# EllarBooher/Syzygy

Measured on AMD Instinct MI355X. Metric: Mpixels/s deferred-lit+atmosphere, higher is better.
Workload: dtype f32

## Files before the change

syzygy_amd/csrc/api_skyview.cpp:

```cpp

#include <new>

#include "api_common.hpp"
#include "lut_state.hpp"
#include "szg/multiscatter_sky.h"

using namespace szg;

struct szg_skyview
{
    int device = 0;
    szg_skyview_desc desc{};
    DeviceBuffer<float> d_transmittance, d_skyview, d_multiscatter, d_aerialLuminance, d_aerialTransmittance;
    float aerialMaxDistance = 0.0f;
    uint32_t multiscatter = SZG_MULTISCATTER_OFF;
    mutable LutState luts;
    DeviceBuffer<unsigned> d_slutStatusAll;
    bool lutReuse = false;
    DeviceBuffer<unsigned> d_lutKey;
    DeviceBuffer<void> d_framePrep;
    DeviceBuffer<void> d_framePrepDraw;
};

static hipError_t ensure_tlut_status(szg_skyview* p, hipStream_t s)
// ... 33 lines not shown

int szg_skyview_create(szg_skyview_t** out, const szg_skyview_desc* desc, int device)
{
    if (out == nullptr)
    {
        return fail(SZG_ERR_INVALID_ARGUMENT, "szg_skyview_create: out is NULL");
    }
    *out = nullptr;
    szg_skyview_desc d{512u, 128u, 2048u, 1024u, 0u, 0u};
    if (desc != nullptr)
    {
        d = *desc;
    }
    if (d.transmittance_width < 2u || d.transmittance_height < 2u || d.skyview_width < 2u || d.skyview_height < 2u ||
        d.transmittance_width > 16384u || d.transmittance_height > 16384u || d.skyview_width > 16384u ||
        d.skyview_height > 16384u)
    {
        return fail(SZG_ERR_INVALID_ARGUMENT, "szg_skyview_create: LUT extents out of range");
    }
    if (d.flags != 0u)
    {
        return fail(SZG_ERR_INVALID_ARGUMENT, "szg_skyview_create: unknown flags 0x%x", d.flags);
    }
    SZG_TRY_RC(select_device(device));
    szg_skyview* p = new (std::nothrow) szg_skyview();
    if (p == nullptr)
    {
        return fail(SZG_ERR_OUT_OF_MEMORY, "szg_skyview_create: host allocation failed");
    }
    p->device = device;
    p->desc = d;
#define SZG_TRY(expr) SZG_HIP_OR(expr, szg_skyview_destroy(p), "szg_skyview_create: hipMalloc")
    size_t const aerialTexels = (size_t)SZG_AERIAL_W * SZG_AERIAL_H * SZG_AERIAL_D;
    SZG_TRY(p->d_transmittance.alloc(tlut_block_bytes(d.transmittance_width, d.transmittance_height) / sizeof(float)));
    SZG_TRY(p->d_skyview.alloc(slut_block_bytes(d.skyview_width, d.skyview_height) / sizeof(float)));
    SZG_TRY(p->d_multiscatter.alloc((size_t)SZG_MULTISCATTER_DIM * SZG_MULTISCATTER_DIM * 4u));
    SZG_TRY(p->d_aerialLuminance.alloc(aerialTexels * 4u));
    SZG_TRY(p->d_aerialTransmittance.alloc(aerialTexels * 4u));
    SZG_TRY(p->d_lutKey.alloc(LUT_KEY_DWORDS, true));
    SZG_TRY(p->d_framePrep.alloc(frame_prep_bytes()));
    SZG_TRY(p->d_slutStatusAll.alloc(SLUT_STATUS_RANKS));
    SZG_TRY(p->d_framePrepDraw.alloc(frame_prep_bytes()));
#undef SZG_TRY
    *out = p;
    return SZG_OK;
}

int szg_skyview_set_lut_reuse(szg_skyview_t* p, int enable)
{
    if (p == nullptr)
    {
        return fail(SZG_ERR_INVALID_ARGUMENT, "szg_skyview_set_lut_reuse: NULL argument");
    }
    p->lutReuse = enable != 0;
    p->luts.reuse_switched();
    return SZG_OK;
}

int szg_skyview_set_multiscatter(szg_skyview_t* p, uint32_t mode)
{
    if (p == nullptr || mode > SZG_MULTISCATTER_ONLY)
    {
        return fail(SZG_ERR_INVALID_ARGUMENT, "szg_skyview_set_multiscatter: NULL pipeline or unknown mode %u", mode);
    }
    if (mode != p->multiscatter)
    {
        p->multiscatter = mode;
// ... 48 lines not shown
    *out = make_image(p->d_transmittance, p->desc.transmittance_width, p->desc.transmittance_height, SZG_FORMAT_RGBA32_SFLOAT);
    p->luts.transmittance_exposed();
    return SZG_OK;
}

int szg_skyview_skyview_lut(const szg_skyview_t* p, szg_image* out)
{
    if (p == nullptr || out == nullptr)
    {
        return fail(SZG_ERR_INVALID_ARGUMENT, "szg_skyview_skyview_lut: NULL argument");
    }
    *out = make_image(p->d_skyview, p->desc.skyview_width, p->desc.skyview_height, SZG_FORMAT_RGBA32_SFLOAT);
    p->luts.skyview_exposed();
    return SZG_OK;
}

int szg_skyview_record_transmittance(szg_skyview_t* p, void* stream, uint32_t atmosphere_index,
                                     const szg_atmosphere_packed* d_atmospheres)
{
    if (p == nullptr || d_atmospheres == nullptr)
    {
        return fail(SZG_ERR_INVALID_ARGUMENT, "szg_skyview_record_transmittance: NULL argument");
    }
    DeviceGuard const guard(p->device);
    hipStream_t const s = static_cast<hipStream_t>(stream);
    const unsigned* dirty = nullptr;
    if (p->lutReuse)
    {
        SZG_HIP(szg::launch_lut_key(s, d_atmospheres, atmosphere_index, nullptr, 0u, p->d_lutKey, 0u, p->luts.forceTransmittance,
                                    p->d_transmittance, p->desc.transmittance_width, p->desc.transmittance_height));
        dirty = p->d_lutKey + 69;
    }
    SZG_HIP(szg::launch_transmittance(s, d_atmospheres, atmosphere_index, p->d_transmittance, p->desc.transmittance_width,
                                      p->desc.transmittance_height, dirty));
    p->luts.transmittance_recorded();
    return SZG_OK;
}

int szg_skyview_record_skyview_lut_rows(szg_skyview_t* p, void* stream, uint32_t atmosphere_index,
                                        const szg_atmosphere_packed* d_atmospheres, uint32_t view_camera_index,
                                        const szg_camera_packed* d_cameras, uint32_t row_begin, uint32_t row_end)
{
    if (p == nullptr || d_atmospheres == nullptr || d_cameras == nullptr)
    {
        return fail(SZG_ERR_INVALID_ARGUMENT, "szg_skyview_record_skyview_lut_rows: NULL argument");
    }
    if (row_begin > row_end || row_end > p->desc.skyview_height)
    {
        return fail(SZG_ERR_INVALID_ARGUMENT, "szg_skyview_record_skyview_lut_rows: rows [%u, %u) outside the %u-row LUT", row_begin,
                    row_end, p->desc.skyview_height);
    }
    if (!multiscatter_ready(p, "szg_skyview_record_skyview_lut_rows"))
    {
        return SZG_ERR_INVALID_ARGUMENT;
    }
    DeviceGuard const guard(p->device);
    hipStream_t const s = static_cast<hipStream_t>(stream);
    bool const whole = LutState::whole(row_begin, row_end, p->desc.skyview_height);
    SZG_HIP(ensure_tlut_status(p, s));
    const unsigned* dirty = nullptr;
    if (p->lutReuse && whole)
    {
        SZG_HIP(szg::launch_lut_key(s, d_atmospheres, atmosphere_index, d_cameras, view_camera_index, p->d_lutKey, 1u, p->luts.forceSkyview,
                                    p->d_skyview, p->desc.skyview_width, p->desc.skyview_height));
        dirty = p->d_lutKey + 70;
    }
    SZG_HIP(szg::launch_frame_prep(s, d_atmospheres, atmosphere_index, p->desc.transmittance_width, p->desc.transmittance_height,
                                   p->d_framePrep));
    if (p->multiscatter == SZG_MULTISCATTER_OFF)
    {
        SZG_HIP(szg::launch_skyview(s, d_atmospheres, atmosphere_index, d_cameras, view_camera_index, p->d_transmittance,
                                    p->desc.transmittance_width, p->desc.transmittance_height, p->d_skyview, p->desc.skyview_width,
                                    p->desc.skyview_height, row_begin, row_end, dirty, p->d_framePrep));
    }
    else
    {
        SZG_HIP(szg::launch_skyview_ms(s, p->multiscatter, d_atmospheres, atmosphere_index, d_cameras, view_camera_index,
                                       p->d_transmittance, p->desc.transmittance_width, p->desc.transmittance_height,
                                       p->d_multiscatter, p->d_skyview, p->desc.skyview_width, p->desc.skyview_height, row_begin,
                                       row_end, dirty, p->d_framePrep));
    }
    p->luts.skyview_rows_recorded(row_begin, row_end, p->desc.skyview_height);
    return SZG_OK;
}

int szg_skyview_lut_row_slice(const szg_skyview_t* p, uint32_t rank, uint32_t nranks, uint32_t* row_begin, uint32_t* row_end)
{
    if (p == nullptr || row_begin == nullptr || row_end == nullptr || nranks == 0u || rank >= nranks)
    {
        return fail(SZG_ERR_INVALID_ARGUMENT, "szg_skyview_lut_row_slice: NULL argument or rank outside [0, nranks)");
    }
    if (p->desc.skyview_height % nranks != 0u)
    {
        return fail(SZG_ERR_INVALID_ARGUMENT, "szg_skyview_lut_row_slice: %u LUT rows do not divide over %u ranks", p->desc.skyview_height,
                    nranks);
    }
    uint32_t const n = p->desc.skyview_height / nranks;
    *row_begin = rank * n;
    *row_end = (rank + 1u) * n;
    return SZG_OK;
}

int szg_skyview_allgather_lut_rows(szg_skyview_t* p, szg_rowtile_comm_t* comm, void* stream)
{
    if (p == nullptr || comm == nullptr)
    {
        return fail(SZG_ERR_INVALID_ARGUMENT, "szg_skyview_allgather_lut_rows: NULL argument");
    }
    int const nranks = szg_rowtile_comm_size(comm);
    if (nranks < 1 || p->desc.skyview_height % (uint32_t)nranks != 0u)
    {
        return fail(SZG_ERR_INVALID_ARGUMENT, "szg_skyview_allgather_lut_rows: %u LUT rows do not divide over %d ranks",
                    p->desc.skyview_height, nranks);
// ... 212 lines not shown
```

syzygy_amd/csrc/kernels_lut.hip:

```cpp

#include "szg/fpmath.h"
#include "szg_atmosphere.hpp"
#include "szg_launch.hpp"
#include "szg_lean.hpp"
#include "szg_lut_rays.hpp"
#include "szg_march.hpp"
#include "szg_vec.hpp"

namespace szg
{
template <int CTRL> SZG_DEV float dpp(float v)
{
    return __builtin_bit_cast(float, __builtin_amdgcn_update_dpp(0, __builtin_bit_cast(int, v), CTRL, 0xF, 0xF, false));
}

constexpr int T_LANES = 8;
constexpr int T_STEPS = 500;

template <bool LEAN> SZG_DEV V3 transmittanceProduct(const Atm& a, V3 origin, V3 direction, float distance, float ndt, int sub)
{
    V3 T = splat(1.0f);
    float const rcp500 = rcpN(500.0f);
#pragma unroll 1
    for (int k = 0; k < (T_STEPS + T_LANES - 1) / T_LANES; k++)
    {
        int const i = k * T_LANES + sub;
        float const t = divRX<LEAN>(distance * ((float)i + 0.5f), 500.0f, rcp500);
        V3 const position = origin + t * direction;
        float const altitude = sqrtPX<LEAN>(dotT(position, position)) - a.planetRadius;
        Extinction const e = sampleExtinction<LEAN>(a, altitude);
        bool const valid = i < T_STEPS;
        float const fx = valid ? expX<LEAN>(ndt * e.extinction.x) : 1.0f;
        float const fy = valid ? expX<LEAN>(ndt * e.extinction.y) : 1.0f;
        float const fz = valid ? expX<LEAN>(ndt * e.extinction.z) : 1.0f;
        T.x = dpp<0x107>(T.x) * fx;
        T.y = dpp<0x107>(T.y) * fy;
        T.z = dpp<0x107>(T.z) * fz;
#pragma unroll
        for (int j = 1; j < T_LANES; j++)
        {
            T.x = dpp<0x111>(T.x) * fx;
            T.y = dpp<0x111>(T.y) * fy;
            T.z = dpp<0x111>(T.z) * fz;
        }
    }
    return T;
}

__global__ __launch_bounds__(256) void k_transmittance(const szg_atmosphere_packed* __restrict__ atmospheres,
                                                      unsigned atmosphereIndex, float4* __restrict__ lut, int W, int H,
                                                      const unsigned* __restrict__ dirty)
{
    if (dirty != nullptr && dirty[0] == 0u)
    {
        return;
    }
    int const sub = (int)(threadIdx.x & (unsigned)(T_LANES - 1));
    int const idRaw = (int)((blockIdx.x * 256u + threadIdx.x) / (unsigned)T_LANES);
    bool const inRangeTexel = idRaw < W * H;
    int const id = inRangeTexel ? idRaw : (W * H - 1);
    int const tx = id % W;
    int const ty = id / W;
    Atm const a = load_atm(atmospheres + atmosphereIndex);

    float const u = ((float)tx + 0.5f) / (float)W;
    float const v = ((float)ty + 0.5f) / (float)H;

    float const x_mu = (u - 0.5f / (float)W) / (1.0f - 1.0f / (float)W);
    float const x_radius = (v - 0.5f / (float)H) / (1.0f - 1.0f / (float)H);
    float const rho = a.H * x_radius;
    float const radius = sqrtf(rho * rho + a.Rp2);
    float const d_min = a.atmosphereRadius - radius;
    float const d_max = rho + a.H;
    float const d = (d_max - d_min) * x_mu + d_min;
    float mu = 1.0f;
    if (d != 0.0f)
    {
        mu = clampf((a.H * a.H - rho * rho - d * d) / (2.0f * radius * d), -1.0f, 1.0f);
    }

    V3 const origin = mk3(0.0f, radius, 0.0f);
    V3 const direction = mk3(sqrtf(1.0f - mu * mu), mu, 0.0f);

    float t0 = 0.0f, t1 = 0.0f;
    bool const hit = raySphere(origin, direction, a.atmosphereRadius, t0, t1);
    float const distance = hit ? t1 : 0.0f;
    float const dt = distance / 500.0f;
    float const ndt = -fabsf(dt);
    float const rmin2 = mu < 0.0f ? radius * radius * (1.0f - mu * mu) : radius * radius;
    bool const lean = waveAll(a.lean && rmin2 >= a.leanFloor2 && inRange(radius, 0x1p-30f, 0x1p30f) && inRange(distance, 0.0f, 0x1p30f));
    V3 const T = lean ? transmittanceProduct<true>(a, origin, direction, distance, ndt, sub)
                      : transmittanceProduct<false>(a, origin, direction, distance, ndt, sub);
    if (inRangeTexel && sub == T_LANES - 1)
    {
        float4 const texel = hit ? make_float4(T.x, T.y, T.z, 1.0f) : make_float4(1.0f, 1.0f, 1.0f, 1.0f);
        lut[id] = texel;
        if (!tlutTexelModerate(texel.x, texel.y, texel.z))
        {
            atomicOr(reinterpret_cast<unsigned*>(lut + (size_t)W * (size_t)H), 1u);
        }
    }
}

__global__ __launch_bounds__(256) void k_lut_range(float4* __restrict__ lut, unsigned n)
{
    unsigned const id = blockIdx.x * 256u + threadIdx.x;
    bool ok = true;
    if (id < n)
    {
        float4 const t = lut[id];
        ok = tlutTexelModerate(t.x, t.y, t.z);
    }
    if (!waveAll(ok) && (threadIdx.x & 63u) == 0u)
    {
        atomicOr(reinterpret_cast<unsigned*>(lut + n), 1u);
    }
}

__global__ __launch_bounds__(64) void k_frame_prep(const szg_atmosphere_packed* __restrict__ atmospheres, unsigned atmosphereIndex,
                                                   int tW, int tH, FramePrep* __restrict__ out,
                                                   const szg_directional_light_packed* __restrict__ sun,
                                                   const szg_camera_packed* __restrict__ cameras, unsigned cameraIndex, unsigned drawW,
                                                   unsigned drawH)
{
    if (threadIdx.x != 0u)
    {
        return;
    }
    FramePrep f{};
    f.a = load_atm(atmospheres + atmosphereIndex);
    f.fwidth = (float)tW;
    f.fheight = (float)tH;
    f.u_bias = 0.5f / (float)tW;
    f.u_scale = 1.0f - 1.0f / (float)tW;
    f.v_bias = 0.5f / (float)tH;
    f.v_scale = 1.0f - 1.0f / (float)tH;
    {
        auto vOf = [&](float x_radius) {
            float const t = SZG_CON(SZG_C_LUTMAP, x_radius, f.v_scale, f.v_bias);
            return SZG_CON(SZG_C_TEXCOORD, t, f.fheight, -0.5f);
        };
        float const rMax = sqrtf(f.a.innerCeil2) * (1.0f + 0x1p-16f);
        float const rhoMax = safeSqrt(rMax * rMax - f.a.Rp2);
        float const vLo = vOf(0.0f), vHi = vOf(rhoMax / f.a.H);
        bool const ok = f.a.lean && vLo >= 0.0f && floorf(vHi) + 1.0f <= f.fheight - 1.0f && vHi == vHi && tW >= 2 && tH >= 2 &&
                        (float)tW * (float)tH <= 0x1p24f;
        f.rowsInterior = ok ? 1u : 0u;
    }
#pragma unroll
    for (int k = 0; k < 16; k++)
    {
        f.sunShadow[k] = 0.0f;
    }
    if (sun != nullptr)
    {
        M4 toTex;
        float const t[16] = {0.5f, 0.0f, 0.0f, 0.0f, 0.0f, 0.5f, 0.0f, 0.0f, 0.0f, 0.0f, 1.0f, 0.0f, 0.5f, 0.5f, 0.0f, 1.0f};
#pragma unroll
        for (int k = 0; k < 16; k++)
        {
// ... 15 lines not shown
        position.y *= -1.0f;
        position.y += f.a.planetRadius;
        c.position = position;
        c.r2 = dot(position, position);
        c.sinHorizon = f.a.planetRadius / length(position);
        c.horizonZenith = PI - szg_asinf(c.sinHorizon);
        c.cosHorizonZenith = -safeSqrt(1.0f - c.sinHorizon * c.sinHorizon);
        c.piMinusHorizon = PI - c.horizonZenith;
        V3 const directionToSun = -f.a.incidentDirectionSun;
        c.projectedLight = normalize(V2{-f.a.incidentDirectionSun.x, -f.a.incidentDirectionSun.z});
        c.sunLength = length(directionToSun);
        c.lightDirection = normalize(directionToSun);
        TLut L{};
        L.width = tW;
        L.height = tH;
        L.fwidth = f.fwidth;
        L.fheight = f.fheight;
        L.u_bias = f.u_bias;
        L.u_scale = f.u_scale;
        L.v_bias = f.v_bias;
        L.v_scale = f.v_scale;
        c.lenFrom = lengthA(position);
        RadiusPart const p = radiusPart<false>(L, f.a, c.lenFrom);
        c.from_r2 = p.r2;
        c.from_d_min = p.d_min;
        c.from_denom = p.denom;
        c.from_rcpDenom = rcpN(p.denom);
        c.from_b = p.b;
        c.from_omb = p.omb;
        c.from_row0 = p.row0;
        c.from_row1 = p.row1;
        c.rcpDrawW = rcpN((float)drawW);
        c.rcpDrawH = rcpN((float)drawH);
    }
    *out = f;
}

__global__ __launch_bounds__(256, 4) void k_skyview(const szg_atmosphere_packed* __restrict__ atmospheres, unsigned atmosphereIndex,
                                                 const szg_camera_packed* __restrict__ cameras, unsigned cameraIndex,
                                                 const float4* __restrict__ tlut, int tW, int tH, float4* __restrict__ lut,
                                                 int W, int H, int rowBegin, int rowEnd, const unsigned* __restrict__ dirty,
                                                 const FramePrep* __restrict__ prep)
{
    if (dirty != nullptr && dirty[0] == 0u)
    {
        return;
    }
    unsigned const tid = threadIdx.x;
    unsigned const wave = tid >> 6, lane = tid & 63u;
    int const x = (int)(blockIdx.x * 32u + wave * 8u + (lane & 7u));
    int const y = rowBegin + (int)(blockIdx.y * 8u + (lane >> 3));
    if (x >= W || y >= rowEnd)
    {
        return;
    }
    Atm const a = load_atm(*prep);
    TLut const L = make_tlut(tlut, tW, tH, *prep);
    const szg_camera_packed* cam = cameras + cameraIndex;
    V3 origin, direction;
    skyviewTexelRay(a, cam, x, y, W, H, origin, direction);

    float const distance = raycastAtmosphere(a, origin, direction);
    V3 const luminance = scatteringIntegral(L, a, origin, direction, distance);
    lut[y * W + x] = make_float4(luminance.x, luminance.y, luminance.z, 1.0f);
    if (!slutTexelFinite(luminance.x, luminance.y, luminance.z))
    {
        atomicOr(reinterpret_cast<unsigned*>(lut + (size_t)W * (size_t)H), 1u);
    }
}

__global__ __launch_bounds__(256) void k_slut_check(float4* __restrict__ lut, unsigned n)
{
    unsigned const id = blockIdx.x * 256u + threadIdx.x;
    bool ok = true;
    if (id < n)
    {
        float4 const t = lut[id];
        ok = slutTexelFinite(t.x, t.y, t.z);
    }
    if (!waveAll(ok) && (threadIdx.x & 63u) == 0u)
    {
        atomicOr(reinterpret_cast<unsigned*>(lut + n), 1u);
    }
}

__global__ void k_slut_status_stage(unsigned* __restrict__ all, unsigned rank, const unsigned* __restrict__ status, unsigned known)
{
    if (threadIdx.x == 0u)
    {
        all[rank] = known != 0u ? status[0] : 1u;
    }
}
__global__ void k_slut_status_reduce(const unsigned* __restrict__ all, unsigned nranks, unsigned* __restrict__ status)
// ... 105 lines not shown
    {
        V3 const pg = pos + tMax * dir;
        V3 const n = normalize(pg);
        float const NdotL = clampf(dot(n, sunDir), 0.0f, 1.0f);
        float const rg = length(pg);
        float const mu_g = dot(pg, sunDir) / rg;
        float const sin_hz = a.planetRadius / rg;
        float const cos_hz = -safeSqrt(1.0f - sin_hz * sin_hz);
        V3 const T_sun = sampleT_RadiusMu(L, a, rg, mu_g) * smoothstep(-sin_hz * sin_sunRadius, sin_hz * sin_sunRadius, mu_g - cos_hz * cos_sunRadius);
        L2 = L2 + Tacc * T_sun * (NdotL * (0.4f / PI));
    }
    V3 const sumL = mk3(waveSum64(L2.x), waveSum64(L2.y), waveSum64(L2.z));
    V3 const sumF = mk3(waveSum64(fms.x), waveSum64(fms.y), waveSum64(fms.z));
    if (lane == 0u)
    {
        V3 const meanL = sumL / 64.0f;
        V3 const meanF = sumF / 64.0f;
        V3 const psi = meanL / (splat(1.0f) - meanF);
        out[ty * dim + tx] = make_float4(psi.x, psi.y, psi.z, 1.0f);
    }
}

hipError_t launch_multiscatter(hipStream_t s, const szg_atmosphere_packed* d_atm, unsigned atmIndex, const float* tlut, unsigned tW,
                               unsigned tH, float* out, unsigned dim)
{
    hipLaunchKernelGGL(k_multiscatter, dim3(dim, dim), dim3(64), 0, s, d_atm, atmIndex, reinterpret_cast<const float4*>(tlut), (int)tW,
                       (int)tH, reinterpret_cast<float4*>(out), dim);
    return hipGetLastError();
}

hipError_t launch_transmittance(hipStream_t s, const szg_atmosphere_packed* d_atm, unsigned atmIndex, float* lut, unsigned W,
                                unsigned H, const unsigned* d_dirty)
{
    unsigned const n = W * H * (unsigned)T_LANES;
    if (d_dirty == nullptr)
    {
        hipError_t const e = hipMemsetAsync(lut + (size_t)W * H * 4u, 0, 4u, s);
        if (e != hipSuccess)
        {
            return e;
        }
    }
    hipLaunchKernelGGL(k_transmittance, dim3((n + 255u) / 256u), dim3(256), 0, s, d_atm, atmIndex, reinterpret_cast<float4*>(lut),
                       (int)W, (int)H, d_dirty);
    return hipGetLastError();
}

__global__ __launch_bounds__(64) void k_lut_key(const szg_atmosphere_packed* __restrict__ atmospheres, unsigned atmosphereIndex,
                                                const szg_camera_packed* __restrict__ cameras, unsigned cameraIndex,
                                                unsigned* __restrict__ state, unsigned which, unsigned force,
                                                unsigned* __restrict__ statusDword)
{
    unsigned const lane = threadIdx.x;
    const unsigned* const atm = reinterpret_cast<const unsigned*>(atmospheres + atmosphereIndex);
    unsigned* const key = state + (which == 0u ? 0u : 32u);
    bool differs = false;
    unsigned mine = 0u;
    if (lane < 32u)
    {
        mine = atm[lane];
        differs = mine != key[lane];
    }
    else if (which == 1u && lane < 35u)
    {
        mine = reinterpret_cast<const unsigned*>((cameras + cameraIndex)->position)[lane - 32u];
        differs = mine != state[64u + (lane - 32u)];
    }
    bool dirty = force != 0u || __builtin_amdgcn_ballot_w64(differs) != 0ull;
    if (which == 1u)
    {
        dirty = dirty || state[67] != state[68];
    }
    if (dirty)
    {
        if (lane < 32u)
        {
            key[lane] = mine;
// ... 4 lines not shown
        }
    }
    if (lane == 0u)
    {
        if (dirty)
        {
            if (which == 0u)
            {
                state[67] = state[67] + 1u;
            }
            else
            {
                state[68] = state[67];
            }
            statusDword[0] = 0u;
        }
        state[69u + which] = dirty ? 1u : 0u;
    }
}

hipError_t launch_lut_key(hipStream_t s, const szg_atmosphere_packed* d_atm, unsigned atmIndex, const szg_camera_packed* d_cam,
                          unsigned camIndex, unsigned* d_state, unsigned which, bool force, float* lutBlock, unsigned W, unsigned H)
{
    hipLaunchKernelGGL(k_lut_key, dim3(1), dim3(64), 0, s, d_atm, atmIndex, d_cam, camIndex, d_state, which, force ? 1u : 0u,
                       reinterpret_cast<unsigned*>(lutBlock + (size_t)W * H * 4u));
    return hipGetLastError();
}

size_t frame_prep_bytes() { return sizeof(FramePrep); }
hipError_t launch_frame_prep(hipStream_t s, const szg_atmosphere_packed* d_atm, unsigned atmIndex, unsigned tW, unsigned tH, void* d_prep,
                             const szg_directional_light_packed* d_sun, const szg_camera_packed* d_cam, unsigned camIndex, unsigned drawW,
                             unsigned drawH)
{
    hipLaunchKernelGGL(k_frame_prep, dim3(1), dim3(64), 0, s, d_atm, atmIndex, (int)tW, (int)tH, static_cast<FramePrep*>(d_prep), d_sun,
                       d_cam, camIndex, drawW, drawH);
    return hipGetLastError();
}

hipError_t launch_lut_range(hipStream_t s, float* lut, unsigned W, unsigned H)
{
    unsigned const n = W * H;
    hipError_t const e = hipMemsetAsync(lut + (size_t)n * 4u, 0, 4u, s);
    if (e != hipSuccess)
    {
        return e;
    }
    hipLaunchKernelGGL(k_lut_range, dim3((n + 255u) / 256u), dim3(256), 0, s, reinterpret_cast<float4*>(lut), n);
    return hipGetLastError();
}

hipError_t launch_slut_check(hipStream_t s, float* lut, unsigned W, unsigned H)
{
    unsigned const n = W * H;
    hipError_t const e = hipMemsetAsync(lut + (size_t)n * 4u, 0, 4, s);
    if (e != hipSuccess)
    {
        return e;
    }
    hipLaunchKernelGGL(k_slut_check, dim3((n + 255u) / 256u), dim3(256), 0, s, reinterpret_cast<float4*>(lut), n);
    return hipGetLastError();
}

hipError_t launch_slut_status_stage(hipStream_t s, unsigned* d_all, unsigned rank, const float* lut, unsigned W, unsigned H, bool known)
{
    hipLaunchKernelGGL(k_slut_status_stage, dim3(1), dim3(64), 0, s, d_all, rank,
                       reinterpret_cast<const unsigned*>(lut + (size_t)W * H * 4u), known ? 1u : 0u);
    return hipGetLastError();
}
hipError_t launch_slut_status_reduce(hipStream_t s, const unsigned* d_all, unsigned nranks, float* lut, unsigned W, unsigned H)
{
    hipLaunchKernelGGL(k_slut_status_reduce, dim3(1), dim3(64), 0, s, d_all, nranks, reinterpret_cast<unsigned*>(lut + (size_t)W * H * 4u));
    return hipGetLastError();
}

hipError_t launch_skyview(hipStream_t s, const szg_atmosphere_packed* d_atm, unsigned atmIndex, const szg_camera_packed* d_cam,
                          unsigned camIndex, const float* tlut, unsigned tW, unsigned tH, float* lut, unsigned W, unsigned H,
                          unsigned rowBegin, unsigned rowEnd, const unsigned* d_dirty, const void* d_prep)
{
    if (rowEnd > H)
    {
        rowEnd = H;
    }
    if (rowBegin >= rowEnd || W == 0u)
    {
        return hipSuccess;
    }
    if (d_dirty == nullptr)
    {
        hipError_t const e = hipMemsetAsync(lut + (size_t)W * H * 4u, 0, 4, s);
        if (e != hipSuccess)
        {
            return e;
        }
    }
    dim3 const grid((W + 31u) / 32u, (rowEnd - rowBegin + 7u) / 8u);
    hipLaunchKernelGGL(k_skyview, grid, dim3(256), 0, s, d_atm, atmIndex, d_cam, camIndex, reinterpret_cast<const float4*>(tlut),
                       (int)tW, (int)tH, reinterpret_cast<float4*>(lut), (int)W, (int)H, (int)rowBegin, (int)rowEnd, d_dirty,
                       static_cast<const FramePrep*>(d_prep));
    return hipGetLastError();
}
}
```

syzygy_amd/csrc/kernels_lut_ms.hip:

```cpp

#include "szg/fpmath.h"
#include "szg/multiscatter_sky.h"
#include "szg_atmosphere.hpp"
#include "szg_launch.hpp"
#include "szg_lean.hpp"
#include "szg_lut_rays.hpp"
#include "szg_march.hpp"
#include "szg_vec.hpp"

#ifndef SZG_MS_STAGE_LDS
#define SZG_MS_STAGE_LDS 0
#endif

namespace szg
{
constexpr unsigned MS_TEXELS = SZG_MULTISCATTER_DIM * SZG_MULTISCATTER_DIM;

template <int MS, bool STAGED>
__global__ __launch_bounds__(256) void k_skyview_ms(const szg_atmosphere_packed* __restrict__ atmospheres, unsigned atmosphereIndex,
                                                    const szg_camera_packed* __restrict__ cameras, unsigned cameraIndex,
                                                    const float4* __restrict__ tlut, int tW, int tH,
                                                    const float4* __restrict__ psi, float4* __restrict__ lut, int W, int H,
                                                    int rowBegin, int rowEnd, const unsigned* __restrict__ dirty,
                                                    const FramePrep* __restrict__ prep)
{
    __shared__ float4 s_psi[STAGED ? MS_TEXELS : 1u];
    if (dirty != nullptr && dirty[0] == 0u)
    {
        return;
    }
    unsigned const tid = threadIdx.x;
    if (STAGED)
    {
#pragma unroll
        for (unsigned k = 0; k < MS_TEXELS / 256u; k++)
        {
            s_psi[k * 256u + tid] = psi[k * 256u + tid];
        }
        __syncthreads();
    }
    unsigned const wave = tid >> 6, lane = tid & 63u;
    int const x = (int)(blockIdx.x * 32u + wave * 8u + (lane & 7u));
    int const y = rowBegin + (int)(blockIdx.y * 8u + (lane >> 3));
    if (x >= W || y >= rowEnd)
    {
        return;
    }
    Atm const a = load_atm(*prep);
    TLut const L = make_tlut(tlut, tW, tH, *prep);
    V3 origin, direction;
    skyviewTexelRay(a, cameras + cameraIndex, x, y, W, H, origin, direction);

    float const distance = raycastAtmosphere(a, origin, direction);
    V3 const luminance = scatteringIntegral<MS>(L, a, origin, direction, distance, STAGED ? s_psi : psi);
    lut[y * W + x] = make_float4(luminance.x, luminance.y, luminance.z, 1.0f);
    if (!slutTexelFinite(luminance.x, luminance.y, luminance.z))
    {
        atomicOr(reinterpret_cast<unsigned*>(lut + (size_t)W * (size_t)H), 1u);
    }
}

template <int MS>
__global__ __launch_bounds__(256) void k_aerial_lut_ms(const szg_atmosphere_packed* __restrict__ atmospheres, unsigned atmosphereIndex,
                                                       const szg_camera_packed* __restrict__ cameras, unsigned cameraIndex,
                                                       const float4* __restrict__ tlut, int tW, int tH,
                                                       const float4* __restrict__ psi, float4* __restrict__ luminance,
                                                       float4* __restrict__ transmittance, unsigned W, unsigned H, unsigned D,
                                                       float maxDistance)
{
    unsigned const id = blockIdx.x * 256u + threadIdx.x;
    if (id >= W * H * D)
    {
        return;
    }
    unsigned const i = id % W, j = (id / W) % H, k = id / (W * H);
    Atm const a = load_atm(atmospheres + atmosphereIndex);
    TLut const L = make_tlut(tlut, tW, tH);
    V3 position, direction;
    aerialFroxelRay(a, cameras + cameraIndex, i, j, W, H, position, direction);

    float const d = (((float)k + 0.5f) / (float)D) * maxDistance;
    V3 const lum = scatteringIntegral<MS>(L, a, position, direction, d, psi);
    V3 const T = sampleT_Segment(L, a, position, position + d * direction);
    luminance[id] = make_float4(lum.x, lum.y, lum.z, 1.0f);
    transmittance[id] = make_float4(T.x, T.y, T.z, 1.0f);
}

template <int MS>
static hipError_t skyview_ms(hipStream_t s, const szg_atmosphere_packed* d_atm, unsigned atmIndex, const szg_camera_packed* d_cam,
                             unsigned camIndex, const float* tlut, unsigned tW, unsigned tH, const float* psi, float* lut, unsigned W,
                             unsigned H, unsigned rowBegin, unsigned rowEnd, const unsigned* d_dirty, const void* d_prep)
{
    dim3 const grid((W + 31u) / 32u, (rowEnd - rowBegin + 7u) / 8u);
    hipLaunchKernelGGL((k_skyview_ms<MS, SZG_MS_STAGE_LDS != 0>), grid, dim3(256), 0, s, d_atm, atmIndex, d_cam, camIndex,
                       reinterpret_cast<const float4*>(tlut), (int)tW, (int)tH, reinterpret_cast<const float4*>(psi),
                       reinterpret_cast<float4*>(lut), (int)W, (int)H, (int)rowBegin, (int)rowEnd, d_dirty,
                       static_cast<const FramePrep*>(d_prep));
    return hipGetLastError();
}

hipError_t launch_skyview_ms(hipStream_t s, unsigned mode, const szg_atmosphere_packed* d_atm, unsigned atmIndex,
                             const szg_camera_packed* d_cam, unsigned camIndex, const float* tlut, unsigned tW, unsigned tH,
                             const float* psi, float* lut, unsigned W, unsigned H, unsigned rowBegin, unsigned rowEnd,
                             const unsigned* d_dirty, const void* d_prep)
{
    if (mode != SZG_MULTISCATTER_ADD && mode != SZG_MULTISCATTER_ONLY)
    {
        return hipErrorInvalidValue;
    }
    if (rowEnd > H)
    {
        rowEnd = H;
    }
    if (rowBegin >= rowEnd || W == 0u)
    {
        return hipSuccess;
    }
    if (d_dirty == nullptr)
    {
        hipError_t const e = hipMemsetAsync(lut + (size_t)W * H * 4u, 0, 4, s);
        if (e != hipSuccess)
        {
            return e;
        }
    }
    return mode == SZG_MULTISCATTER_ADD
               ? skyview_ms<1>(s, d_atm, atmIndex, d_cam, camIndex, tlut, tW, tH, psi, lut, W, H, rowBegin, rowEnd, d_dirty, d_prep)
               : skyview_ms<2>(s, d_atm, atmIndex, d_cam, camIndex, tlut, tW, tH, psi, lut, W, H, rowBegin, rowEnd, d_dirty, d_prep);
}

hipError_t launch_aerial_lut_ms(hipStream_t s, unsigned mode, const szg_atmosphere_packed* d_atm, unsigned atmIndex,
                                const szg_camera_packed* d_cam, unsigned camIndex, const float* tlut, unsigned tW, unsigned tH,
                                const float* psi, float* luminance, float* transmittance, unsigned W, unsigned H, unsigned D,
                                float maxDistance)
{
    if (mode != SZG_MULTISCATTER_ADD && mode != SZG_MULTISCATTER_ONLY)
    {
        return hipErrorInvalidValue;
    }
    unsigned const n = W * H * D;
    dim3 const grid((n + 255u) / 256u);
    if (mode == SZG_MULTISCATTER_ADD)
    {
        hipLaunchKernelGGL(k_aerial_lut_ms<1>, grid, dim3(256), 0, s, d_atm, atmIndex, d_cam, camIndex,
                           reinterpret_cast<const float4*>(tlut), (int)tW, (int)tH, reinterpret_cast<const float4*>(psi),
                           reinterpret_cast<float4*>(luminance), reinterpret_cast<float4*>(transmittance), W, H, D, maxDistance);
    }
    else
    {
        hipLaunchKernelGGL(k_aerial_lut_ms<2>, grid, dim3(256), 0, s, d_atm, atmIndex, d_cam, camIndex,
                           reinterpret_cast<const float4*>(tlut), (int)tW, (int)tH, reinterpret_cast<const float4*>(psi),
// ... 6 lines not shown
```

syzygy_amd/csrc/szg_atmosphere.hpp:

```cpp
#pragma once

#include "szg/abi.h"
#include "szg/fpmath.h"
#include "szg_lean.hpp"
#include "szg_vec.hpp"

namespace szg
{
struct Atm
{
    V3 scatteringRayleigh;
    float densityScaleRayleigh;
    V3 absorptionRayleigh;
    float planetRadius;
    V3 scatteringMie;
    float densityScaleMie;
    float atmosphereRadius;
    V3 incidentDirectionSun;
    V3 scatteringOzone;
    V3 absorptionOzone;
    V3 sunIntensitySpectrum;
    float sunAngularRadius;
    float Ra2, Rp2, H;
    float rcpH, rcpDsR, rcpDsM, rcp15;
// ... 207 lines not shown
    TLut t;
    t.moderate = reinterpret_cast<const unsigned*>(texels + (size_t)w * (size_t)h)[0] == 0u;
    t.texels = texels;
    t.width = w;
    t.height = h;
    t.fwidth = (float)w;
    t.fheight = (float)h;
    t.u_bias = 0.5f / (float)w;
    t.u_scale = 1.0f - 1.0f / (float)w;
    t.v_bias = 0.5f / (float)h;
    t.v_scale = 1.0f - 1.0f / (float)h;
    t.rowsInterior = false;
    return t;
}

struct FramePrep
{
    Atm a;
    float fwidth, fheight, u_bias, u_scale, v_bias, v_scale;
    float sunShadow[16];
    unsigned rowsInterior;
    struct Camera
    {
        V3 position;
        float r2, sinHorizon;
        float horizonZenith, cosHorizonZenith, piMinusHorizon;
        V2 projectedLight;
        float sunLength;
        V3 lightDirection;
        float lenFrom, from_r2, from_d_min, from_denom, from_rcpDenom, from_b, from_omb;
        unsigned from_row0, from_row1;
        float rcpDrawW, rcpDrawH;
    } camera;
};
SZG_DEV float inVector(float x)
{
    asm volatile("" : "+v"(x));
    return x;
}
SZG_DEV V3 inVector(V3 v) { return V3{inVector(v.x), inVector(v.y), inVector(v.z)}; }
SZG_DEV Atm load_atm(const FramePrep& f)
{
    Atm a = f.a;
    a.scatteringRayleigh = inVector(a.scatteringRayleigh);
    a.densityScaleRayleigh = inVector(a.densityScaleRayleigh);
    a.absorptionRayleigh = inVector(a.absorptionRayleigh);
    a.planetRadius = inVector(a.planetRadius);
    a.scatteringMie = inVector(a.scatteringMie);
    a.densityScaleMie = inVector(a.densityScaleMie);
    a.atmosphereRadius = inVector(a.atmosphereRadius);
    a.incidentDirectionSun = inVector(a.incidentDirectionSun);
    a.scatteringOzone = inVector(a.scatteringOzone);
    a.absorptionOzone = inVector(a.absorptionOzone);
    a.sunIntensitySpectrum = inVector(a.sunIntensitySpectrum);
    a.sunAngularRadius = inVector(a.sunAngularRadius);
    a.Ra2 = inVector(a.Ra2);
    a.Rp2 = inVector(a.Rp2);
    a.H = inVector(a.H);
    a.rcpH = inVector(a.rcpH);
    a.rcpDsR = inVector(a.rcpDsR);
    a.rcpDsM = inVector(a.rcpDsM);
    a.rcp15 = inVector(a.rcp15);
    a.leanFloor2 = inVector(a.leanFloor2);
    a.extFloor2 = inVector(a.extFloor2);
    a.extCeil2 = inVector(a.extCeil2);
    a.innerCeil2 = inVector(a.innerCeil2);
// ... 231 lines not shown
```

syzygy_amd/csrc/szg_launch.hpp:

```cpp
#pragma once

#include <hip/hip_runtime_api.h>

#include "szg/abi.h"
#include "szg/compute_collection.h"
#include "szg/debuglines.h"
#include "szg/present.h"
#include "szg/raster.h"
#include "szg/texture_display.h"
#include "szg/ui_layer.h"

namespace szg
{
struct LightRec
{
    float shadowRows[16];
    float dir[3];
    float falloffFactor;
    float colorStrength[3];
    float falloffDistance;
    float position[3];
    unsigned isSpot;
    const float* map;
    unsigned mapWidth, mapHeight;
    unsigned mapPitchFloats;
    unsigned leanOK;
    float falloffBound;
    float rcpFalloffDistance;
};
static_assert(sizeof(LightRec) == 144, "LightRec layout");

struct ShadowSlot
{
    const float* map;
    unsigned width, height, pitchFloats, pad;
};
static_assert(sizeof(ShadowSlot) == 24, "ShadowSlot layout");

struct AerialLut
{
    const float* luminance;
    unsigned W, H, D;
    float maxDistance;
};

struct TileArgs
{
    unsigned block_rows, rank, nranks, local_rows;
};

inline size_t tlut_block_bytes(unsigned W, unsigned H) { return (size_t)W * H * 16u + 16u; }
hipError_t launch_lut_range(hipStream_t s, float* lut, unsigned W, unsigned H);
hipError_t launch_transmittance(hipStream_t s, const szg_atmosphere_packed* d_atm, unsigned atmIndex, float* lut, unsigned W,
                                unsigned H, const unsigned* d_dirty = nullptr);
constexpr unsigned LUT_KEY_DWORDS = 72u;
constexpr unsigned SLUT_STATUS_RANKS = 64u;
hipError_t launch_lut_key(hipStream_t s, const szg_atmosphere_packed* d_atm, unsigned atmIndex, const szg_camera_packed* d_cam,
                          unsigned camIndex, unsigned* d_state, unsigned which, bool force, float* lutBlock, unsigned W, unsigned H);
inline size_t slut_block_bytes(unsigned W, unsigned H) { return (size_t)W * H * 16u + 16u; }
hipError_t launch_slut_check(hipStream_t s, float* lut, unsigned W, unsigned H);
hipError_t launch_slut_status_stage(hipStream_t s, unsigned* d_all, unsigned rank, const float* lut, unsigned W, unsigned H, bool known);
hipError_t launch_slut_status_reduce(hipStream_t s, const unsigned* d_all, unsigned nranks, float* lut, unsigned W, unsigned H);
hipError_t launch_skyview(hipStream_t s, const szg_atmosphere_packed* d_atm, unsigned atmIndex, const szg_camera_packed* d_cam,
                          unsigned camIndex, const float* tlut, unsigned tW, unsigned tH, float* lut, unsigned W, unsigned H,
                          unsigned rowBegin, unsigned rowEnd, const unsigned* d_dirty, const void* d_prep);
size_t frame_prep_bytes();
hipError_t launch_frame_prep(hipStream_t s, const szg_atmosphere_packed* d_atm, unsigned atmIndex, unsigned tW, unsigned tH, void* d_prep,
                             const szg_directional_light_packed* d_sun = nullptr, const szg_camera_packed* d_cam = nullptr,
                             unsigned camIndex = 0u, unsigned drawW = 0u, unsigned drawH = 0u);
hipError_t launch_composite(hipStream_t s, const szg_scene_texture& scene, unsigned drawW, unsigned drawH, TileArgs tile,
                            const szg_gbuffer& g, ShadowSlot sunSlot, const szg_atmosphere_packed* d_atm, unsigned atmIndex, const szg_camera_packed* d_cam,
                            unsigned camIndex, const szg_directional_light_packed* d_dir, unsigned sunIndex, const float* tlut,
                            unsigned tW, unsigned tH, const float* slut, unsigned sW, unsigned sH, AerialLut aerial, const void* d_prep);
hipError_t launch_aerial_lut(hipStream_t s, const szg_atmosphere_packed* d_atm, unsigned atmIndex, const szg_camera_packed* d_cam,
                             unsigned camIndex, const float* tlut, unsigned tW, unsigned tH, float* luminance, float* transmittance,
                             unsigned W, unsigned H, unsigned D, float maxDistance);
hipError_t launch_multiscatter(hipStream_t s, const szg_atmosphere_packed* d_atm, unsigned atmIndex, const float* tlut, unsigned tW,
                               unsigned tH, float* out, unsigned dim);
hipError_t launch_skyview_ms(hipStream_t s, unsigned mode, const szg_atmosphere_packed* d_atm, unsigned atmIndex,
                             const szg_camera_packed* d_cam, unsigned camIndex, const float* tlut, unsigned tW, unsigned tH,
                             const float* psi, float* lut, unsigned W, unsigned H, unsigned rowBegin, unsigned rowEnd,
                             const unsigned* d_dirty, const void* d_prep);
hipError_t launch_aerial_lut_ms(hipStream_t s, unsigned mode, const szg_atmosphere_packed* d_atm, unsigned atmIndex,
                                const szg_camera_packed* d_cam, unsigned camIndex, const float* tlut, unsigned tW, unsigned tH,
                                const float* psi, float* luminance, float* transmittance, unsigned W, unsigned H, unsigned D,
                                float maxDistance);

hipError_t launch_light_prep(hipStream_t s, const szg_directional_light_packed* d_dir, unsigned dirCount, unsigned dirSkip,
                             const szg_spot_light_packed* d_spot, unsigned spotCount, const ShadowSlot* d_slots,
                             unsigned slotCount, LightRec* d_out);
hipError_t launch_lights(hipStream_t s, const szg_scene_texture& scene, unsigned drawW, unsigned drawH, TileArgs tile,
                         const szg_gbuffer& g, const szg_camera_packed* d_cam, unsigned camIndex, const LightRec* d_lights,
                         unsigned lightCount, const unsigned long long* d_tileMasks);
hipError_t launch_light_tiles(hipStream_t s, unsigned drawW, unsigned drawH, TileArgs tile, const szg_gbuffer& g,
                              const LightRec* d_lights, unsigned lightCount, unsigned long long* d_tileMasks);

hipError_t launch_gbuffer_fill(hipStream_t s, const szg_scene_texture& scene, unsigned drawW, unsigned drawH, TileArgs tile,
                               const szg_gbuffer& g, const szg_camera_packed* d_cam, unsigned camIndex, float ground_y,
                               float ground_half_extent, float checker_cell, float ground_roughness,
                               const szg_fill_box* d_boxes, unsigned boxCount);
struct ShadowGen
{
    float projView[16];
    float invProjView[16];
    float* map;
    unsigned dim, pitchFloats, pad;
};
hipError_t launch_shadow_maps(hipStream_t s, const szg_directional_light_packed* d_dir, unsigned dirCount,
                              const szg_spot_light_packed* d_spot, unsigned spotCount, const ShadowSlot* d_ownedSlots,
                              unsigned slotCount, ShadowGen* d_gen, const szg_fill_box* d_boxes, unsigned boxCount, unsigned maxDim);
hipError_t launch_shadow_prep(hipStream_t s, const szg_directional_light_packed* d_dir, unsigned dirCount,
                              const szg_spot_light_packed* d_spot, unsigned spotCount, const ShadowSlot* d_ownedSlots,
                              unsigned slotCount, ShadowGen* d_gen);

hipError_t launch_oetf_table(hipStream_t s, unsigned short* table, unsigned function);
// ... 142 lines not shown
```

syzygy_amd/csrc/szg_lut_rays.hpp:

```cpp
#pragma once

#include "szg/fpmath.h"
#include "szg_atmosphere.hpp"
#include "szg_vec.hpp"

namespace szg
{
SZG_DEV void skyviewTexelRay(const Atm& a, const szg_camera_packed* cam, int x, int y, int W, int H, V3& origin, V3& direction)
{
    float const PI = 3.141592653589793f;

    float const u = ((float)x + 0.5f) / (float)W;
    float const v = ((float)y + 0.5f) / (float)H;

    origin = mk3(cam->position[0], cam->position[1], cam->position[2]) / 1000000.0f;
    origin.y *= -1.0f;
    origin.y += a.planetRadius;

    float const radius = length(origin);
    float const sinHorizonZenith = a.planetRadius / radius;
    float const horizonZenith = PI - szg_asinf(sinHorizonZenith);
    float const cosineViewLightProjected = (u - 0.5f) * 2.0f;
    V2 const lightDirectionProjected = normalize(V2{-a.incidentDirectionSun.x, -a.incidentDirectionSun.z});
    float azimuthSun = szg_asinf(lightDirectionProjected.x);
    if (lightDirectionProjected.y < 0.0f)
    {
        azimuthSun = PI - azimuthSun;
    }
    float const azimuth = szg_acosf(clampf(cosineViewLightProjected, -1.0f, 1.0f)) + azimuthSun;
    float viewZenith;
    float const unnormalized_v = 2.0f * v - 1.0f;
    if (v < 0.5f)
    {
        float const angleFraction = 1.0f - unnormalized_v * unnormalized_v;
        viewZenith = angleFraction * horizonZenith;
    }
    else
    {
        float const angleFraction = unnormalized_v * unnormalized_v;
        viewZenith = (PI - horizonZenith) * angleFraction + horizonZenith;
    }
    float const elevation = -(viewZenith - PI / 2.0f);

    float const ce = szg_cosf(elevation);
    direction = normalize(mk3(szg_sinf(azimuth) * ce, szg_sinf(elevation), szg_cosf(azimuth) * ce));
}

SZG_DEV void aerialFroxelRay(const Atm& a, const szg_camera_packed* cam, unsigned i, unsigned j, unsigned W, unsigned H, V3& position,
                             V3& direction)
{
    position = mk3(cam->position[0], cam->position[1], cam->position[2]) / 1000000.0f;
    position.y *= -1.0f;
    position.y += a.planetRadius;
    float const clipx = (((float)i + 0.5f) / (float)W - 0.5f) * 2.0f;
    float const clipy = (((float)j + 0.5f) / (float)H - 0.5f) * 2.0f;
    V4 const dvs = mul(load_m4(cam->inverseProjection), clipx, clipy, 1.0f, 1.0f);
    V4 const rot = mul(load_m4(cam->rotation), dvs.x, dvs.y, dvs.z, dvs.w);
    direction = normalize(mk3(rot.x, rot.y, rot.z));
    direction.y *= -1.0f;
}
}
```

Measured before the change: 2586.

## Fold LUT status clears into kernels and hoist sky-ray frame terms into prep

Removes the per-frame hipMemsetAsync status clears before the transmittance and skyview launches. The transmittance kernel now does a grid-wide reduction through zero-initialised counters, and the last block writes the status and resets the counters. The skyview status is cleared inside the frame_prep kernel. Camera-invariant sky-ray terms (origin, horizon zenith, sun azimuth) are computed once in frame_prep instead of per texel. This cuts small launches and per-texel asin work, but adds a block barrier, a ticket atomic per block in the transmittance kernel, and a counter scheme that relies on the transmittance buffer being zeroed at allocation.

After: 2589 (median of 3 runs). No clear change (+0.1%).

```diff
diff --git a/syzygy_amd/csrc/api_skyview.cpp b/syzygy_amd/csrc/api_skyview.cpp
--- a/syzygy_amd/csrc/api_skyview.cpp
+++ b/syzygy_amd/csrc/api_skyview.cpp
@@ -89,7 +89,7 @@
     p->desc = d;
 #define SZG_TRY(expr) SZG_HIP_OR(expr, szg_skyview_destroy(p), "szg_skyview_create: hipMalloc")
     size_t const aerialTexels = (size_t)SZG_AERIAL_W * SZG_AERIAL_H * SZG_AERIAL_D;
-    SZG_TRY(p->d_transmittance.alloc(tlut_block_bytes(d.transmittance_width, d.transmittance_height) / sizeof(float)));
+    SZG_TRY(p->d_transmittance.alloc(tlut_block_bytes(d.transmittance_width, d.transmittance_height) / sizeof(float), true));
     SZG_TRY(p->d_skyview.alloc(slut_block_bytes(d.skyview_width, d.skyview_height) / sizeof(float)));
     SZG_TRY(p->d_multiscatter.alloc((size_t)SZG_MULTISCATTER_DIM * SZG_MULTISCATTER_DIM * 4u));
     SZG_TRY(p->d_aerialLuminance.alloc(aerialTexels * 4u));
@@ -204,7 +204,7 @@
         dirty = p->d_lutKey + 69;
     }
     SZG_HIP(szg::launch_transmittance(s, d_atmospheres, atmosphere_index, p->d_transmittance, p->desc.transmittance_width,
-                                      p->desc.transmittance_height, dirty));
+                                      p->desc.transmittance_height, dirty, true));
     p->luts.transmittance_recorded();
     return SZG_OK;
 }
@@ -237,20 +237,23 @@
                                     p->d_skyview, p->desc.skyview_width, p->desc.skyview_height));
         dirty = p->d_lutKey + 70;
     }
+    bool const prepClears = dirty == nullptr;
+    unsigned* const slutStatus =
+        reinterpret_cast<unsigned*>(p->d_skyview.get() + (size_t)p->desc.skyview_width * p->desc.skyview_height * 4u);
     SZG_HIP(szg::launch_frame_prep(s, d_atmospheres, atmosphere_index, p->desc.transmittance_width, p->desc.transmittance_height,
-                                   p->d_framePrep));
+                                   p->d_framePrep, nullptr, d_cameras, view_camera_index, 0u, 0u, prepClears ? slutStatus : nullptr));
     if (p->multiscatter == SZG_MULTISCATTER_OFF)
     {
         SZG_HIP(szg::launch_skyview(s, d_atmospheres, atmosphere_index, d_cameras, view_camera_index, p->d_transmittance,
                                     p->desc.transmittance_width, p->desc.transmittance_height, p->d_skyview, p->desc.skyview_width,
-                                    p->desc.skyview_height, row_begin, row_end, dirty, p->d_framePrep));
+                                    p->desc.skyview_height, row_begin, row_end, dirty, p->d_framePrep, prepClears));
     }
     else
     {
         SZG_HIP(szg::launch_skyview_ms(s, p->multiscatter, d_atmospheres, atmosphere_index, d_cameras, view_camera_index,
                                        p->d_transmittance, p->desc.transmittance_width, p->desc.transmittance_height,
                                        p->d_multiscatter, p->d_skyview, p->desc.skyview_width, p->desc.skyview_height, row_begin,
-                                       row_end, dirty, p->d_framePrep));
+                                       row_end, dirty, p->d_framePrep, prepClears));
     }
     p->luts.skyview_rows_recorded(row_begin, row_end, p->desc.skyview_height);
     return SZG_OK;
diff --git a/syzygy_amd/csrc/kernels_lut.hip b/syzygy_amd/csrc/kernels_lut.hip
--- a/syzygy_amd/csrc/kernels_lut.hip
+++ b/syzygy_amd/csrc/kernels_lut.hip
@@ -49,7 +49,7 @@
 
 __global__ __launch_bounds__(256) void k_transmittance(const szg_atmosphere_packed* __restrict__ atmospheres,
                                                       unsigned atmosphereIndex, float4* __restrict__ lut, int W, int H,
-                                                      const unsigned* __restrict__ dirty)
+                                                      const unsigned* __restrict__ dirty, unsigned* __restrict__ counters)
 {
     if (dirty != nullptr && dirty[0] == 0u)
     {
@@ -91,13 +91,41 @@
     bool const lean = waveAll(a.lean && rmin2 >= a.leanFloor2 && inRange(radius, 0x1p-30f, 0x1p30f) && inRange(distance, 0.0f, 0x1p30f));
     V3 const T = lean ? transmittanceProduct<true>(a, origin, direction, distance, ndt, sub)
                       : transmittanceProduct<false>(a, origin, direction, distance, ndt, sub);
+    unsigned* const status = reinterpret_cast<unsigned*>(lut + (size_t)W * (size_t)H);
+    bool outOfRange = false;
     if (inRangeTexel && sub == T_LANES - 1)
     {
         float4 const texel = hit ? make_float4(T.x, T.y, T.z, 1.0f) : make_float4(1.0f, 1.0f, 1.0f, 1.0f);
         lut[id] = texel;
-        if (!tlutTexelModerate(texel.x, texel.y, texel.z))
-        {
-            atomicOr(reinterpret_cast<unsigned*>(lut + (size_t)W * (size_t)H), 1u);
+        outOfRange = !tlutTexelModerate(texel.x, texel.y, texel.z);
+        if (outOfRange && counters == nullptr)
+        {
+            atomicOr(status, 1u);
+        }
+    }
+    if (counters == nullptr)
+    {
+        return;
+    }
+    __shared__ unsigned s_outOfRange[4];
+    bool const waveOutOfRange = !waveAll(!outOfRange);
+    if ((threadIdx.x & 63u) == 0u)
+    {
+        s_outOfRange[threadIdx.x >> 6] = waveOutOfRange ? 1u : 0u;
+    }
+    __syncthreads();
+    if (threadIdx.x == 0u)
+    {
+        if ((s_outOfRange[0] | s_outOfRange[1] | s_outOfRange[2] | s_outOfRange[3]) != 0u)
+        {
+            __hip_atomic_fetch_or(&counters[0], 1u, __ATOMIC_RELAXED, __HIP_MEMORY_SCOPE_AGENT);
+        }
+        unsigned const ticket = __hip_atomic_fetch_add(&counters[1], 1u, __ATOMIC_ACQ_REL, __HIP_MEMORY_SCOPE_AGENT);
+        if (ticket == gridDim.x - 1u)
+        {
+            status[0] = __hip_atomic_load(&counters[0], __ATOMIC_RELAXED, __HIP_MEMORY_SCOPE_AGENT);
+            counters[0] = 0u;
+            counters[1] = 0u;
         }
     }
 }
@@ -121,11 +149,15 @@
                                                    int tW, int tH, FramePrep* __restrict__ out,
                                                    const szg_directional_light_packed* __restrict__ sun,
                                                    const szg_camera_packed* __restrict__ cameras, unsigned cameraIndex, unsigned drawW,
-                                                   unsigned drawH)
+                                                   unsigned drawH, unsigned* __restrict__ clearStatus)
 {
     if (threadIdx.x != 0u)
     {
         return;
+    }
+    if (clearStatus != nullptr)
+    {
+        clearStatus[0] = 0u;
     }
     FramePrep f{};
     f.a = load_atm(atmospheres + atmosphereIndex);
@@ -207,6 +239,7 @@
         c.from_row1 = p.row1;
         c.rcpDrawW = rcpN((float)drawW);
         c.rcpDrawH = rcpN((float)drawH);
+        f.skyRay = skyRayFrameTerms(f.a, cam);
     }
     *out = f;
 }
@@ -231,9 +264,8 @@
     }
     Atm const a = load_atm(*prep);
     TLut const L = make_tlut(tlut, tW, tH, *prep);
-    const szg_camera_packed* cam = cameras + cameraIndex;
     V3 origin, direction;
-    skyviewTexelRay(a, cam, x, y, W, H, origin, direction);
+    skyviewTexelRay(prep->skyRay, x, y, W, H, origin, direction);
 
     float const distance = raycastAtmosphere(a, origin, direction);
     V3 const luminance = scatteringIntegral(L, a, origin, direction, distance);
@@ -405,8 +437,15 @@
 hipError_t launch_transmittance(hipStream_t s, const szg_atmosphere_packed* d_atm, unsigned atmIndex, float* lut, unsigned W,
                                 unsigned H, const unsigned* d_dirty)
 {
+    return launch_transmittance(s, d_atm, atmIndex, lut, W, H, d_dirty, false);
+}
+
+hipError_t launch_transmittance(hipStream_t s, const szg_atmosphere_packed* d_atm, unsigned atmIndex, float* lut, unsigned W,
+                                unsigned H, const unsigned* d_dirty, bool countersZeroed)
+{
     unsigned const n = W * H * (unsigned)T_LANES;
-    if (d_dirty == nullptr)
+    unsigned* const status = reinterpret_cast<unsigned*>(lut + (size_t)W * H * 4u);
+    if (d_dirty == nullptr && !countersZeroed)
     {
         hipError_t const e = hipMemsetAsync(lut + (size_t)W * H * 4u, 0, 4u, s);
         if (e != hipSuccess)
@@ -415,7 +454,7 @@
         }
     }
     hipLaunchKernelGGL(k_transmittance, dim3((n + 255u) / 256u), dim3(256), 0, s, d_atm, atmIndex, reinterpret_cast<float4*>(lut),
-                       (int)W, (int)H, d_dirty);
+                       (int)W, (int)H, d_dirty, countersZeroed ? status + 1 : nullptr);
     return hipGetLastError();
 }
 
@@ -486,8 +525,15 @@
                              const szg_directional_light_packed* d_sun, const szg_camera_packed* d_cam, unsigned camIndex, unsigned drawW,
                              unsigned drawH)
 {
+    return launch_frame_prep(s, d_atm, atmIndex, tW, tH, d_prep, d_sun, d_cam, camIndex, drawW, drawH, nullptr);
+}
+
+hipError_t launch_frame_prep(hipStream_t s, const szg_atmosphere_packed* d_atm, unsigned atmIndex, unsigned tW, unsigned tH, void* d_prep,
+                             const szg_directional_light_packed* d_sun, const szg_camera_packed* d_cam, unsigned camIndex, unsigned drawW,
+                             unsigned drawH, unsigned* d_clearStatus)
+{
     hipLaunchKernelGGL(k_frame_prep, dim3(1), dim3(64), 0, s, d_atm, atmIndex, (int)tW, (int)tH, static_cast<FramePrep*>(d_prep), d_sun,
-                       d_cam, camIndex, drawW, drawH);
+                       d_cam, camIndex, drawW, drawH, d_clearStatus);
     return hipGetLastError();
 }
 
@@ -531,6 +577,13 @@
                           unsigned camIndex, const float* tlut, unsigned tW, unsigned tH, float* lut, unsigned W, unsigned H,
                           unsigned rowBegin, unsigned rowEnd, const unsigned* d_dirty, const void* d_prep)
 {
+    return launch_skyview(s, d_atm, atmIndex, d_cam, camIndex, tlut, tW, tH, lut, W, H, rowBegin, rowEnd, d_dirty, d_prep, false);
+}
+
+hipError_t launch_skyview(hipStream_t s, const szg_atmosphere_packed* d_atm, unsigned atmIndex, const szg_camera_packed* d_cam,
+                          unsigned camIndex, const float* tlut, unsigned tW, unsigned tH, float* lut, unsigned W, unsigned H,
+                          unsigned rowBegin, unsigned rowEnd, const unsigned* d_dirty, const void* d_prep, bool statusCleared)
+{
     if (rowEnd > H)
     {
         rowEnd = H;
@@ -539,7 +592,7 @@
     {
         return hipSuccess;
     }
-    if (d_dirty == nullptr)
+    if (d_dirty == nullptr && !statusCleared)
     {
         hipError_t const e = hipMemsetAsync(lut + (size_t)W * H * 4u, 0, 4, s);
         if (e != hipSuccess)
diff --git a/syzygy_amd/csrc/kernels_lut_ms.hip b/syzygy_amd/csrc/kernels_lut_ms.hip
--- a/syzygy_amd/csrc/kernels_lut_ms.hip
+++ b/syzygy_amd/csrc/kernels_lut_ms.hip
@@ -49,7 +49,7 @@
     Atm const a = load_atm(*prep);
     TLut const L = make_tlut(tlut, tW, tH, *prep);
     V3 origin, direction;
-    skyviewTexelRay(a, cameras + cameraIndex, x, y, W, H, origin, direction);
+    skyviewTexelRay(prep->skyRay, x, y, W, H, origin, direction);
 
     float const distance = raycastAtmosphere(a, origin, direction);
     V3 const luminance = scatteringIntegral<MS>(L, a, origin, direction, distance, STAGED ? s_psi : psi);
@@ -104,6 +104,15 @@
                              const float* psi, float* lut, unsigned W, unsigned H, unsigned rowBegin, unsigned rowEnd,
                              const unsigned* d_dirty, const void* d_prep)
 {
+    return launch_skyview_ms(s, mode, d_atm, atmIndex, d_cam, camIndex, tlut, tW, tH, psi, lut, W, H, rowBegin, rowEnd, d_dirty, d_prep,
+                             false);
+}
+
+hipError_t launch_skyview_ms(hipStream_t s, unsigned mode, const szg_atmosphere_packed* d_atm, unsigned atmIndex,
+                             const szg_camera_packed* d_cam, unsigned camIndex, const float* tlut, unsigned tW, unsigned tH,
+                             const float* psi, float* lut, unsigned W, unsigned H, unsigned rowBegin, unsigned rowEnd,
+                             const unsigned* d_dirty, const void* d_prep, bool statusCleared)
+{
     if (mode != SZG_MULTISCATTER_ADD && mode != SZG_MULTISCATTER_ONLY)
     {
         return hipErrorInvalidValue;
@@ -116,7 +125,7 @@
     {
         return hipSuccess;
     }
-    if (d_dirty == nullptr)
+    if (d_dirty == nullptr && !statusCleared)
     {
         hipError_t const e = hipMemsetAsync(lut + (size_t)W * H * 4u, 0, 4, s);
         if (e != hipSuccess)
diff --git a/syzygy_amd/csrc/szg_atmosphere.hpp b/syzygy_amd/csrc/szg_atmosphere.hpp
--- a/syzygy_amd/csrc/szg_atmosphere.hpp
+++ b/syzygy_amd/csrc/szg_atmosphere.hpp
@@ -263,6 +263,13 @@
         unsigned from_row0, from_row1;
         float rcpDrawW, rcpDrawH;
     } camera;
+    struct SkyRay
+    {
+        V3 origin;
+        float horizonZenith;
+        float piMinusHorizon;
+        float azimuthSun;
+    } skyRay;
 };
 SZG_DEV float inVector(float x)
 {
diff --git a/syzygy_amd/csrc/szg_launch.hpp b/syzygy_amd/csrc/szg_launch.hpp
--- a/syzygy_amd/csrc/szg_launch.hpp
+++ b/syzygy_amd/csrc/szg_launch.hpp
@@ -53,6 +53,8 @@
 hipError_t launch_lut_range(hipStream_t s, float* lut, unsigned W, unsigned H);
 hipError_t launch_transmittance(hipStream_t s, const szg_atmosphere_packed* d_atm, unsigned atmIndex, float* lut, unsigned W,
                                 unsigned H, const unsigned* d_dirty = nullptr);
+hipError_t launch_transmittance(hipStream_t s, const szg_atmosphere_packed* d_atm, unsigned atmIndex, float* lut, unsigned W,
+                                unsigned H, const unsigned* d_dirty, bool countersZeroed);
 constexpr unsigned LUT_KEY_DWORDS = 72u;
 constexpr unsigned SLUT_STATUS_RANKS = 64u;
 hipError_t launch_lut_key(hipStream_t s, const szg_atmosphere_packed* d_atm, unsigned atmIndex, const szg_camera_packed* d_cam,
@@ -64,10 +66,16 @@
 hipError_t launch_skyview(hipStream_t s, const szg_atmosphere_packed* d_atm, unsigned atmIndex, const szg_camera_packed* d_cam,
                           unsigned camIndex, const float* tlut, unsigned tW, unsigned tH, float* lut, unsigned W, unsigned H,
                           unsigned rowBegin, unsigned rowEnd, const unsigned* d_dirty, const void* d_prep);
+hipError_t launch_skyview(hipStream_t s, const szg_atmosphere_packed* d_atm, unsigned atmIndex, const szg_camera_packed* d_cam,
+                          unsigned camIndex, const float* tlut, unsigned tW, unsigned tH, float* lut, unsigned W, unsigned H,
+                          unsigned rowBegin, unsigned rowEnd, const unsigned* d_dirty, const void* d_prep, bool statusCleared);
 size_t frame_prep_bytes();
 hipError_t launch_frame_prep(hipStream_t s, const szg_atmosphere_packed* d_atm, unsigned atmIndex, unsigned tW, unsigned tH, void* d_prep,
                              const szg_directional_light_packed* d_sun = nullptr, const szg_camera_packed* d_cam = nullptr,
                              unsigned camIndex = 0u, unsigned drawW = 0u, unsigned drawH = 0u);
+hipError_t launch_frame_prep(hipStream_t s, const szg_atmosphere_packed* d_atm, unsigned atmIndex, unsigned tW, unsigned tH, void* d_prep,
+                             const szg_directional_light_packed* d_sun, const szg_camera_packed* d_cam, unsigned camIndex, unsigned drawW,
+                             unsigned drawH, unsigned* d_clearStatus);
 hipError_t launch_composite(hipStream_t s, const szg_scene_texture& scene, unsigned drawW, unsigned drawH, TileArgs tile,
                             const szg_gbuffer& g, ShadowSlot sunSlot, const szg_atmosphere_packed* d_atm, unsigned atmIndex, const szg_camera_packed* d_cam,
                             unsigned camIndex, const szg_directional_light_packed* d_dir, unsigned sunIndex, const float* tlut,
@@ -81,6 +89,10 @@
                              const szg_camera_packed* d_cam, unsigned camIndex, const float* tlut, unsigned tW, unsigned tH,
                              const float* psi, float* lut, unsigned W, unsigned H, unsigned rowBegin, unsigned rowEnd,
                              const unsigned* d_dirty, const void* d_prep);
+hipError_t launch_skyview_ms(hipStream_t s, unsigned mode, const szg_atmosphere_packed* d_atm, unsigned atmIndex,
+                             const szg_camera_packed* d_cam, unsigned camIndex, const float* tlut, unsigned tW, unsigned tH,
+                             const float* psi, float* lut, unsigned W, unsigned H, unsigned rowBegin, unsigned rowEnd,
+                             const unsigned* d_dirty, const void* d_prep, bool statusCleared);
 hipError_t launch_aerial_lut_ms(hipStream_t s, unsigned mode, const szg_atmosphere_packed* d_atm, unsigned atmIndex,
                                 const szg_camera_packed* d_cam, unsigned camIndex, const float* tlut, unsigned tW, unsigned tH,
                                 const float* psi, float* luminance, float* transmittance, unsigned W, unsigned H, unsigned D,
diff --git a/syzygy_amd/csrc/szg_lut_rays.hpp b/syzygy_amd/csrc/szg_lut_rays.hpp
--- a/syzygy_amd/csrc/szg_lut_rays.hpp
+++ b/syzygy_amd/csrc/szg_lut_rays.hpp
@@ -6,28 +6,41 @@
 
 namespace szg
 {
-SZG_DEV void skyviewTexelRay(const Atm& a, const szg_camera_packed* cam, int x, int y, int W, int H, V3& origin, V3& direction)
+SZG_DEV FramePrep::SkyRay skyRayFrameTerms(const Atm& a, const szg_camera_packed* cam)
+{
+    float const PI = 3.141592653589793f;
+    FramePrep::SkyRay f;
+
+    f.origin = mk3(cam->position[0], cam->position[1], cam->position[2]) / 1000000.0f;
+    f.origin.y *= -1.0f;
+    f.origin.y += a.planetRadius;
+
+    float const radius = length(f.origin);
+    float const sinHorizonZenith = a.planetRadius / radius;
+    f.horizonZenith = PI - szg_asinf(sinHorizonZenith);
+    V2 const lightDirectionProjected = normalize(V2{-a.incidentDirectionSun.x, -a.incidentDirectionSun.z});
+    float azimuthSun = szg_asinf(lightDirectionProjected.x);
+    if (lightDirectionProjected.y < 0.0f)
+    {
+        azimuthSun = PI - azimuthSun;
+    }
+    f.azimuthSun = azimuthSun;
+    f.piMinusHorizon = PI - f.horizonZenith;
+    return f;
+}
+
+SZG_DEV void skyviewTexelRay(const FramePrep::SkyRay& f, int x, int y, int W, int H, V3& origin, V3& direction)
 {
     float const PI = 3.141592653589793f;
 
     float const u = ((float)x + 0.5f) / (float)W;
     float const v = ((float)y + 0.5f) / (float)H;
 
-    origin = mk3(cam->position[0], cam->position[1], cam->position[2]) / 1000000.0f;
-    origin.y *= -1.0f;
-    origin.y += a.planetRadius;
+    origin = inVector(f.origin);
 
-    float const radius = length(origin);
-    float const sinHorizonZenith = a.planetRadius / radius;
-    float const horizonZenith = PI - szg_asinf(sinHorizonZenith);
+    float const horizonZenith = f.horizonZenith;
     float const cosineViewLightProjected = (u - 0.5f) * 2.0f;
-    V2 const lightDirectionProjected = normalize(V2{-a.incidentDirectionSun.x, -a.incidentDirectionSun.z});
-    float azimuthSun = szg_asinf(lightDirectionProjected.x);
-    if (lightDirectionProjected.y < 0.0f)
-    {
-        azimuthSun = PI - azimuthSun;
-    }
-    float const azimuth = szg_acosf(clampf(cosineViewLightProjected, -1.0f, 1.0f)) + azimuthSun;
+    float const azimuth = szg_acosf(clampf(cosineViewLightProjected, -1.0f, 1.0f)) + f.azimuthSun;
     float viewZenith;
     float const unnormalized_v = 2.0f * v - 1.0f;
     if (v < 0.5f)
@@ -38,7 +51,7 @@
     else
     {
         float const angleFraction = unnormalized_v * unnormalized_v;
-        viewZenith = (PI - horizonZenith) * angleFraction + horizonZenith;
+        viewZenith = f.piMinusHorizon * angleFraction + horizonZenith;
     }
     float const elevation = -(viewZenith - PI / 2.0f);
 
```
